# microsoft/Sora

Hardware: AMD Instinct MI355X
Metric: IQ Msamples/s through 802.11a 54 Mbps RX PHY (higher is better)
Workload: dtype int16 IQ / u8 path metrics

## Files before the change

### sora_amd/csrc/dev_vit16.h

```cpp
#pragma once
#include <hip/hip_runtime.h>
#include "kernels.h"
#include "dev_viterbi.h"

namespace sora {
namespace {

template <int WIN, int LOOK> struct Geom16 {
    static constexpr int kMaxWalk = (WIN + LOOK + 7) / 8 + 2;
    static constexpr int P = kMaxWalk;
    static constexpr int kPathBytes = 40;
};

template <int WIN, int LOOK> struct Lds16 {
    uint16_t ring[Geom16<WIN, LOOK>::P][4][64];
    union {
        uint32_t udump[4][64];
        uint16_t ops[4][24][2];
        uint16_t ops2[2][4][24][2];
    };
    uint8_t  path[8][Geom16<WIN, LOOK>::kPathBytes];
};

constexpr unsigned kW[4] = { 0u, 21u, 42u, 63u };

__device__ __forceinline__ unsigned v_of_lane(unsigned l)
{
    const unsigned b0 = l & 1u, b1 = (l >> 1) & 1u, b2 = (l >> 2) & 1u, b3 = (l >> 3) & 1u;
    const unsigned c3 = b2, c1 = b3, c0 = b0 ^ c3, c2 = b1 ^ c3;
    return c0 | (c1 << 1) | (c2 << 2) | (c3 << 3);
}
__device__ __forceinline__ unsigned lane_of_v(unsigned v)
{
    const unsigned c0 = v & 1u, c1 = (v >> 1) & 1u, c2 = (v >> 2) & 1u, c3 = (v >> 3) & 1u;
    return c0 ^ (c2 << 1) ^ (c1 << 3) ^ (c3 ? 7u : 0u);
}
__device__ __forceinline__ unsigned rev6u(unsigned x) { return __brev(x) >> 26; }

template <int CTRL> __device__ __forceinline__ unsigned dppx(unsigned v) { return (unsigned)__builtin_amdgcn_update_dpp(0, (int)v, CTRL, 0xF, 0xF, true); }

__device__ __forceinline__ unsigned partner(unsigned v, int ph)
{
    switch (ph) {
    case 0: return dppx<0x140>(v);
    case 1: return dppx<0x1B>(v);
    case 2: return dppx<0x141>(v);
    case 3: return dppx<0x4E>(v);
    case 4: return dppx<0x128>(v);
    default: return dppx<0xB1>(v);
    }
}

struct Vit16 {
    unsigned U[4];
    unsigned MX[24];
    unsigned MY[6];
    unsigned sadr[3][4];
};

template <int WHICH, int P>
__device__ __forceinline__ void acs16(Vit16& V, int t24, unsigned a, unsigned b, unsigned pos512[3])
{
    const int ph = t24 % 6, k = t24 % 8;
    const unsigned Kp = (WHICH == 0 ? 14u : 7u) * kFld + (kOne << k);
    unsigned bm;
    if (WHICH == 0)      bm = (a ^ V.MX[t24]) + (b ^ V.MY[ph]);
    else if (WHICH == 1) bm = a ^ V.MX[t24];
    else                 bm = b ^ V.MX[t24];
    const unsigned bo = Kp - bm;
    const int rx = ph == 0 ? 2 : ph == 1 ? 1 : 0;
    unsigned N[4];
#pragma unroll
    for (int i = 0; i < 4; i++) {
        const unsigned X = V.U[i], Y = partner(V.U[i ^ rx], ph);
        const bool wb = (kW[i] >> (5 - ph)) & 1u;
        N[i] = wb ? pk_min16(X + bo, Y + bm) : pk_min16(X + bm, Y + bo);
    }
#pragma unroll
    for (int i = 0; i < 4; i++) V.U[i] = N[i];
    if (k == 7) {
        const int jb = t24 / 8;
#pragma unroll
        for (int i = 0; i < 4; i++) {
            const unsigned w = bank_word(V.U[i]);
            const unsigned addr = V.sadr[jb][i] + pos512[jb];
            asm volatile("ds_write_b16 %0, %1" : : "v"(addr), "v"(w) : "memory");
            V.U[i] &= 0xFE00FE00u;
        }
    }
}

__device__ __forceinline__ unsigned row_min_u32(unsigned v)
{
    v = min(v, dppx<0xB1>(v)); v = min(v, dppx<0x4E>(v)); v = min(v, dppx<0x141>(v)); v = min(v, dppx<0x128>(v));
    return v;
}
__device__ __forceinline__ unsigned row_pkmin(unsigned v)
{
    v = pk_min16(v, dppx<0xB1>(v)); v = pk_min16(v, dppx<0x4E>(v)); v = pk_min16(v, dppx<0x141>(v)); v = pk_min16(v, dppx<0x128>(v));
    return v;
}
__device__ __forceinline__ unsigned wave_min_u32(unsigned v) { return (unsigned)__builtin_amdgcn_readfirstlane((int)dpp_min_u32_wave(v)); }
__device__ __forceinline__ unsigned wave_max_u32(unsigned v) { return ~wave_min_u32(~v); }

template <int CR, int WIN, int LOOK, int BITS>
struct Forward16 {
    static constexpr int P = Geom16<WIN, LOOK>::P, GB = Puncture<CR>::GB, GS = Puncture<CR>::GS, CW = Puncture<CR>::CW;
    static constexpr int NV = Puncture<CR>::NV;
    struct Chunk { uint32_t v[CW]; };
    struct Raw { SoftRaw r[NV]; };

    Vit16 V;
    unsigned row, half;
    uint32_t my_j;
    SoftCursor<BITS, CW> cur[NV];
    const uint8_t* soft;
    uint16_t* my_ops;
    const uint4* row_ops;
    uint32_t pos;
    unsigned pos512[3];
    uint32_t tr, nsteps;
    uint32_t next_thr;
    bool all_done;

    __device__ __forceinline__ void init(Lds16<WIN, LOOK>& S, const uint8_t* __restrict__ soft_, uint32_t my_soft_off, uint32_t my_first, uint32_t my_last, unsigned start,
                                         uint32_t nsteps_)
    {
        const unsigned lane = threadIdx.x & 63, l16 = lane & 15;
        row = lane >> 4; half = lane & 1u;
        const unsigned v0 = v_of_lane(l16);
        nsteps = nsteps_;
#pragma unroll
        for (int i = 0; i < 4; i++) V.U[i] = (v0 ^ kW[i]) == 0 ? 0u : start;
        const unsigned ring_base = (unsigned)(uintptr_t)&S.ring[0][0][0];
#pragma unroll
        for (int jb = 0; jb < 3; jb++)
#pragma unroll
            for (int i = 0; i < 4; i++) V.sadr[jb][i] = ring_base + ((row * 64u + rev6u(rol6(v0 ^ kW[i], jb == 0 ? 2 : jb == 1 ? 4 : 0))) << 1);
#pragma unroll
        for (int t = 0; t < 24; t++) {
            const int ph = t % 6, k = t % 8;
            const unsigned n = rol6(v0, ph + 1);
            const bool vb = (v0 >> (5 - ph)) & 1u;
            const unsigned ma = (__popc(n & 0155) & 1) ? 7u * kFld : 0u, mb = (__popc(n & 0117) & 1) ? 7u * kFld : 0u;
            const unsigned mx = Puncture<CR>::which_of(ph) == 2 ? mb : ma;
            V.MX[t] = vb ? ((mx ^ (7u * kFld)) | (kOne << k)) : mx;
            if (t < 6) V.MY[t] = vb ? (mb ^ (7u * kFld)) : mb;
        }
        tr = 0; pos = 0;
        my_j = l16 >> 1;
#pragma unroll
        for (int v = 0; v < NV; v++) cur[v].init(my_soft_off, my_first + my_j + 8u * v, my_last);
        soft = soft_;
        my_ops = &S.ops[row][my_j][half];
        row_ops = reinterpret_cast<const uint4*>(&S.ops[row][0][0]);
        set_row_pos();
    }
    __device__ __forceinline__ bool going() const { return tr < nsteps && !all_done; }

    __device__ __forceinline__ void normalize()
    {
        const unsigned m = row_pkmin(pk_min16(pk_min16(V.U[0], V.U[1]), pk_min16(V.U[2], V.U[3])));
#pragma unroll
        for (int i = 0; i < 4; i++) V.U[i] -= m;
    }
    static __device__ __forceinline__ uint32_t pos_of(uint32_t p, int jb) { const uint32_t q = p + (uint32_t)jb; return q >= (uint32_t)P ? q - (uint32_t)P : q; }
    __device__ __forceinline__ void set_row_pos()
    {
#pragma unroll
        for (int jb = 0; jb < 3; jb++) pos512[jb] = pos_of(pos, jb) * 512u;
    }
    __device__ __forceinline__ void end_row() { pos = pos_of(pos, 3); set_row_pos(); }
    __device__ __forceinline__ Raw fetch(uint32_t c) const
    {
        Raw R;
#pragma unroll
        for (int v = 0; v < NV; v++) R.r[v] = cur[v].fetch(soft, c);
        return R;
    }
    __device__ __forceinline__ void put(const Raw& R, uint16_t* mine) const
    {
#pragma unroll
        for (int v = 0; v < NV; v++) mine[16 * v] = (uint16_t)cur[v].field(R.r[v]);
    }
    static __device__ __forceinline__ Chunk get(const uint4* table)
    {
        Chunk K;
#pragma unroll
        for (int i = 0; i < (CW + 3) / 4; i++) {
            const uint4 x = table[i];
            K.v[4 * i] = x.x; K.v[4 * i + 1] = x.y;
            if (4 * i + 2 < CW) { K.v[4 * i + 2] = x.z; K.v[4 * i + 3] = x.w; }
        }
        return K;
    }
    __device__ __forceinline__ Chunk unpack(const Raw& R) const
    {
        put(R, my_ops);
        lds_fence();
        const Chunk K = get(row_ops);
        lds_fence();
        return K;
    }
    __device__ __forceinline__ void group(const Chunk& K, int h, int i0)
    {
        const int k0 = i0 / GS * GB, t24 = 12 * h + i0;
        acs16<0, P>(V, t24, K.v[k0], K.v[k0 + 1], pos512);
        if (CR != 0) acs16<1, P>(V, t24 + 1, K.v[k0 + 2], 0, pos512);
        if (CR == 2) acs16<2, P>(V, t24 + 2, 0, K.v[k0 + 3], pos512);
        if ((t24 + GS) % 8 == 0) normalize();
    }
    __device__ __forceinline__ void fast_chunk(const Chunk& K, int h)
    {
#pragma unroll
        for (int g = 0; g < 12 / GS; g++) group(K, h, g * GS);
        tr += 12;
    }
    template <typename CHECK> __device__ __forceinline__ void slow_chunk(const Chunk& K, int h, CHECK& check)
    {
#pragma unroll
        for (int g = 0; g < 12 / GS; g++) {
            if (going()) {
                group(K, h, g * GS);
                tr += GS;
                check(12 * h + g * GS + GS - 1);
            }
        }
    }
    template <typename CHECK> __device__ __forceinline__ void chunk(const Chunk& K, int h, CHECK& check)
    {
        if (tr + 12 <= nsteps && next_thr > tr + 12) fast_chunk(K, h); else slow_chunk(K, h, check);
    }
};

template <int WIN, int LOOK, bool LANE_OB = false>
__device__ __noinline__ void trace16(unsigned lds_off, unsigned U0, unsigned U1, unsigned U2, unsigned U3, uint32_t tr_, uint32_t ob_, uint32_t pj_, uint32_t k_,
                                     uint32_t my_cnt, uint8_t* my_out)
{
    using G = Geom16<WIN, LOOK>;
    constexpr int P = G::P;
    typedef __attribute__((address_space(3))) Lds16<WIN, LOOK> lds_t;
    lds_t& S = *(lds_t*)(uintptr_t)lds_off;
    auto uni = [](uint32_t v) { return (uint32_t)__builtin_amdgcn_readfirstlane((int)v); };
    const uint32_t tr = uni(tr_), ob = LANE_OB ? ob_ : uni(ob_), pj = uni(pj_), k = uni(k_);
    const unsigned lane = threadIdx.x & 63, row = lane >> 4, l16 = lane & 15, half = lane & 1u;
    const unsigned v0 = v_of_lane(l16);
    const unsigned U[4] = { U0, U1, U2, U3 };
    const uint32_t j = (tr - 1) >> 3, nn = tr - 8u * j, m_lo = ob >> 3;
#pragma unroll
    for (int i = 0; i < 4; i++) S.udump[i][lane] = U[i];
    lds_fence();
    unsigned key[2] = { 0xFFFFFFFFu, 0xFFFFFFFFu };
#pragma unroll
    for (int i = 0; i < 4; i++) {
        const unsigned st = rol6(v0 ^ kW[i], tr);
        unsigned lastA, lastB;
        if (k == 7) { const unsigned w = S.ring[pj][row][rev6u(st)]; lastA = (w >> 7) & 1u; lastB = (w >> 15) & 1u; }
        else { lastA = (U[i] >> k) & 1u; lastB = (U[i] >> (17 + k)) & 1u; }
        const unsigned mA = ((U[i] & 0xFFFFu) >> 9 << 1) | lastA, mB = (U[i] >> 25 << 1) | lastB;
        key[0] = min(key[0], (mA << 8) | (st << 2)); key[1] = min(key[1], (mB << 8) | (st << 2));
    }
    const unsigned kA = row_min_u32(key[0]), kB = row_min_u32(key[1]);
    const unsigned st = ((half ? kB : kA) >> 2) & 0x3Fu;
    const unsigned s0 = rol6(st, 6u - tr % 6u);
    const unsigned b4 = (s0 >> 4) & 1u, b5 = (s0 >> 5) & 1u;
    const unsigned ri = b4 | (b5 << 1);
    const unsigned sl = lane_of_v((s0 ^ (b4 ? 21u : 0u) ^ (b5 ? 42u : 0u)) & 15u);
    const unsigned Ust = S.udump[ri][row * 16u + sl];
    unsigned H;
    if (nn == 8) H = ((unsigned)S.ring[pj][row][rev6u(st)] >> (8u * half)) & 0xFFu;
    else H = ((Ust >> (17u * half)) & 0xFFu) & ((1u << nn) - 1u);
    unsigned q = rev6u(((st >> nn) | rev6u(H & 0x3Fu)) & 0x3Fu);
    __attribute__((address_space(3))) uint8_t* pth = S.path[row * 2u + half];
    pth[0] = (uint8_t)H;
    typedef __attribute__((address_space(3))) const uint16_t lds_u16;
    const unsigned rowbase = (unsigned)(uintptr_t)&S.ring[0][row][0], sh = 8u * half;
#pragma unroll
    for (int i = 1; i < G::kMaxWalk; i++) {
        const int d = (int)pj - i;
        const uint32_t p = (uint32_t)(d < 0 ? d + P : d);
        unsigned base = rowbase + p * 512u;
        asm volatile("" : "+v"(base));
        const unsigned raw = *(lds_u16*)(uintptr_t)(base + (q << 1));
        pth[i] = (uint8_t)(raw >> sh);
        q = __builtin_amdgcn_ubfe(raw, sh, 6u);
    }
    lds_fence();
    const uint32_t nbytes = my_cnt >> 3;
    for (uint32_t z = l16 >> 1; z < nbytes; z += 8) {
        const uint32_t m = m_lo + z, i1 = j - m;
        my_out[m] = (uint8_t)(((unsigned)pth[i1] >> 6) | (((unsigned)pth[i1 - 1] & 0x3Fu) << 2));
    }
    lds_fence();
}

}
}
```

### sora_amd/csrc/k_rx.hip

```cpp
#include <hip/hip_runtime.h>
#include <utility>
#include "kernels.h"
#include "dev_sym11a.h"
#include "dev_viterbi.h"
#include "dev_winplan.h"
#include "dev_vitwin.h"

namespace sora {

struct FrameLds {
    uint32_t eq[4][4][64];
    uint8_t  soft[4][4][288];
    uint8_t  demap[1024];
    int4     trk[4][4];
    int      nsym_of[4];
    short    st0[4][4];
};
template <bool SHARED>
__device__ __forceinline__ void frame_symbols(const RxArgs& A, uint32_t j, FrameLds& lds, bool valid = true)
{
    uint32_t (&s_eq)[4][4][64] = lds.eq; uint8_t (&s_soft)[4][4][288] = lds.soft; const uint8_t* s_demap = lds.demap;
    const int w = threadIdx.x >> 6, lane = threadIdx.x & 63, g = lane >> 4, e = lane & 15;
    const Tables& T = A.T;
    const uint32_t f = valid ? A.joblist[j] : 0u;
    FrameRow r = A.frames[f];
    if (!valid) { r.nsym = 0; r.nbpsc = 1; }
    if (lane == 0 && valid) A.jobs[j] = frame_vitjob(r);
    const FrameCtx* fx = A.fctx + f;
    const uint32_t* iq = A.iq + A.caps[r.capture].offset;
    const Fft64TwPk W = fft64_twiddles_pk(T, e);
    PkTw fq[4], ch[4];
#pragma unroll
    for (int m = 0; m < 4; m++) { fq[m] = pk_tw_mul(fx->freq[e + 16 * m]); ch[m] = pk_tw_mul(fx->chan[e + 16 * m]); }
    const int nb = __builtin_amdgcn_readfirstlane((int)r.nbpsc), ncbps = 48 * nb, nsym = __builtin_amdgcn_readfirstlane((int)r.nsym);
    uint32_t mp[4];
    const bool packs = deint_packs(nb, lane);
    deint_map_words(T, nb, lane, mp);
    uint8_t* dst = A.soft + (size_t)r.slot0 * kSoftBytesPerSlot;
    const int pk = lane & 3;
    const int pbin = pk == 0 ? 43 : pk == 1 ? 57 : pk == 2 ? 7 : 21, pc = pk == 0 ? -21 : pk == 1 ? -7 : pk == 2 ? 7 : 21;
    int cfo_comp = r.cfo_comp, sfo_comp = r.sfo_comp, cfo_tr = r.cfo_tracker, sfo_tr = r.sfo_tracker;
    unsigned symbol_count = 0;

    auto load_samples = [&](int s0, uint32_t raw[4]) {
        const uint32_t p0 = r.data_start + 80u * (uint32_t)(s0 + g) + 8u;
#pragma unroll
        for (int m = 0; m < 4; m++) raw[m] = (s0 + g <= nsym) ? iq[(size_t)(p0 + (uint32_t)(e + 16 * m)) * A.str] : 0u;
    };
    int nsym_loop = nsym, nsym_f = nsym;
    if (SHARED) {
        if (lane == 0) { lds.nsym_of[w] = nsym; lds.st0[w][0] = (short)cfo_comp; lds.st0[w][1] = (short)sfo_comp; lds.st0[w][2] = (short)cfo_tr; lds.st0[w][3] = (short)sfo_tr; }
        __syncthreads();
        nsym_loop = max(max(lds.nsym_of[0], lds.nsym_of[1]), max(lds.nsym_of[2], lds.nsym_of[3]));
        const int fr = (lane >> 2) & 3;
        nsym_f = lds.nsym_of[fr];
        cfo_comp = lds.st0[fr][0]; sfo_comp = lds.st0[fr][1]; cfo_tr = lds.st0[fr][2]; sfo_tr = lds.st0[fr][3];
    }
    uint32_t raw[4];
    load_samples(1, raw);
    for (int s0 = 1; s0 <= nsym_loop; s0 += 4) {
        const int sym = s0 + g;
        const bool active = sym <= nsym;
        const bool mine = s0 <= nsym;
        int4 rec = { 0, 0, 0, 0 };
        if (mine) {
            pcx x[4], Y[4];
#pragma unroll
            for (int m = 0; m < 4; m++) x[m] = sym_freq_comp(raw[m], fq[m]);
            if (s0 + 4 <= nsym) load_samples(s0 + 4, raw);
            fft64_core_pk(x, s_eq[w][g], e, W, wave_lds_sync);
#pragma unroll
            for (int q = 0; q < 4; q++) Y[q] = s_eq[w][g][__brev((unsigned)(e + 16 * q)) >> 26];
            wave_lds_sync();
#pragma unroll
            for (int q = 0; q < 4; q++) s_eq[w][g][e + 16 * q] = sym_equalise(Y[q], ch[q], e + 16 * q);
            wave_lds_sync();
        }
        if (SHARED) {
            __syncthreads();
            if (w == 0) {
                const int fr = (lane >> 2) & 3;
#pragma unroll
                for (int gg = 0; gg < 4; gg++) {
                    const cpx p = mul_q15(unpack(s_eq[fr][gg][pbin]), rot_coeff(T, w16(cfo_comp + pc * sfo_comp)));
                    const int th = pilot_angle(pk == 3 ? uatan2(T, -p.im, -p.re) : uatan2(T, p.im, p.re), (symbol_count + (unsigned)gg) % 127u);
                    int th1 = __builtin_amdgcn_update_dpp(0, th, 0x00, 0xF, 0xF, true), th2 = __builtin_amdgcn_update_dpp(0, th, 0x55, 0xF, 0xF, true);
                    int th3 = __builtin_amdgcn_update_dpp(0, th, 0xAA, 0xF, 0xF, true), th4 = __builtin_amdgcn_update_dpp(0, th, 0xFF, 0xF, 0xF, true);
                    asm volatile("" : "+v"(th1), "+v"(th2), "+v"(th3), "+v"(th4));
                    const int4 t = track_advance(th1, th2, th3, th4, s0 + gg <= nsym_f, cfo_comp, sfo_comp, cfo_tr, sfo_tr);
                    if (lane < 16 && pk == 0) lds.trk[fr][gg] = t;
                }
            }
            symbol_count = (symbol_count + 4u) % 127u;
            __syncthreads();
            rec = lds.trk[w][g];
        } else {
            int4 t[4];
#pragma unroll
            for (int gg = 0; gg < 4; gg++) {
                t[gg] = int4{ cfo_comp, sfo_comp, 0, 0 };
                if (s0 + gg <= nsym) {
                    const cpx p = mul_q15(unpack(s_eq[w][gg][pbin]), rot_coeff(T, w16(cfo_comp + pc * sfo_comp)));
                    const int th = pilot_angle(pk == 3 ? uatan2(T, -p.im, -p.re) : uatan2(T, p.im, p.re), symbol_count);
                    symbol_count++; if (symbol_count >= 127) symbol_count = 0;
                    t[gg] = track_advance(__builtin_amdgcn_readlane(th, 0), __builtin_amdgcn_readlane(th, 1), __builtin_amdgcn_readlane(th, 2), __builtin_amdgcn_readlane(th, 3),
                                          true, cfo_comp, sfo_comp, cfo_tr, sfo_tr);
                }
            }
            rec = t[0];
            if (g == 1) rec = t[1]; else if (g == 2) rec = t[2]; else if (g == 3) rec = t[3];
        }
        if (!mine) continue;
        if (active) {
            uint32_t v3[3];
#pragma unroll
            for (int m = 0; m < 3; m++) v3[m] = s_eq[w][g][carrier_bin48(e + 16 * m)];
            sym_back_demap(T, s_demap, v3, rec, nb, e, s_soft[w][g]);
        }
        wave_lds_sync();
        {
            const int nact = min(4, nsym - s0 + 1);
            const uint32_t sym_bytes = 3u * (uint32_t)ncbps / 8u;
            uint8_t* d = dst + (size_t)(s0 - 1) * sym_bytes;
            for (int gs = 0; gs < nact; gs++, d += sym_bytes)
                if (packs) soft3_store8(d, (uint32_t)lane, deint_gather24(s_soft[w][gs], mp));
        }
        wave_lds_sync();
    }
}
__global__ void __launch_bounds__(256) k_frame(RxArgs A)
{
    __shared__ FrameLds lds;
    reinterpret_cast<uint32_t*>(lds.demap)[threadIdx.x] = reinterpret_cast<const uint32_t*>(A.T.demap)[threadIdx.x];
    __syncthreads();
    if (!locate_job(blockIdx.x * 4, A.njobs).ok) return;
    const JobRef jr = locate_job(blockIdx.x * 4 + (threadIdx.x >> 6), A.njobs);
    frame_symbols<true>(A, jr.ok ? jr.list * A.nrows + jr.idx : 0u, lds, jr.ok);
}

typedef uint32_t u32x4_t __attribute__((ext_vector_type(4)));
__device__ __forceinline__ void store16_through(uint4* p, uint4 v)
{
    const u32x4_t x = { v.x, v.y, v.z, v.w };
    asm volatile("global_store_dwordx4 %0, %1, off sc1\n\ts_nop 1" : : "v"(p), "v"(x) : "memory");
}
__device__ __forceinline__ void store4_through(uint32_t* p, uint32_t v) { __hip_atomic_store(p, v, __ATOMIC_RELAXED, __HIP_MEMORY_SCOPE_AGENT); }

template <bool THROUGH>
__device__ __forceinline__ void sym_front_block(const RxArgs& A, uint32_t bid, uint32_t (*s_eq)[4][64])
{
    const int w = threadIdx.x >> 6, lane = threadIdx.x & 63, g = lane >> 4, e = lane & 15;
    const Tables& T = A.T;
    const WaveSlots S = wave_slots(A, bid);
    if (S.owned == 0) return;
    uint32_t own[kSlotIters];
#pragma unroll
    for (int it = 0; it < kSlotIters; it++) own[it] = S.owner(it, g);
    const Fft64TwPk W = fft64_twiddles_pk(T, e);
    uint32_t* sl = s_eq[w][g];
    uint4* eq4 = reinterpret_cast<uint4*>(A.eq);
    auto store = [&](uint32_t slot, const uint32_t o[4]) {
        if (THROUGH) store16_through(eq4 + ((size_t)slot * 16u + (uint32_t)e), uint4{ o[0], o[1], o[2], o[3] });
        else eq4[(size_t)slot * 16u + (uint32_t)e] = uint4{ o[0], o[1], o[2], o[3] };
        auto pilot = [&](uint32_t k, uint32_t v) { if (THROUGH) store4_through(A.pil + ((size_t)slot * 4u + k), v); else A.pil[(size_t)slot * 4u + k] = v; };
        if (e == 10) pilot(0u, o[3]);
        if (e == 14) pilot(1u, o[1]);
        if (e == 1)  pilot(2u, o[3]);
        if (e == 5)  pilot(3u, o[1]);
    };
    if (S.one_frame) {
        const FrameRow& r = A.frames[S.row0];
        const uint32_t* iq = A.iq + A.caps[r.capture].offset;
        const uint32_t ds = r.data_start, s0 = r.slot0, str = A.str;
        const FrameCtx* fx = A.fctx + S.row0;
        uint32_t raw[kSlotIters][4];
#pragma unroll
        for (int it = 0; it < kSlotIters; it++) {
            const uint32_t p0 = ds + 80u * (S.slot(it, g) - s0) + 8u;
#pragma unroll
            for (int m = 0; m < 4; m++) raw[it][m] = own[it] != kNoOwner ? iq[(size_t)(p0 + (uint32_t)(e + 16 * m)) * str] : 0u;
        }
        PkTw fq[4], ch[4];
#pragma unroll
        for (int m = 0; m < 4; m++) { fq[m] = pk_tw_mul(fx->freq[e + 16 * m]); ch[m] = pk_tw_mul(fx->chan[4 * e + m]); }
#pragma unroll
        for (int it = 0; it < kSlotIters; it++) {
            if (S.quad(it) == 0) continue;
            uint32_t o[4];
            sym_front_quad(raw[it], fq, ch, sl, e, W, o);
            if (own[it] != kNoOwner) store(S.slot(it, g), o);
        }
        return;
    }
#pragma unroll 1
    for (int it = 0; it < kSlotIters; it++) {
        if (S.quad(it) == 0) continue;
        const uint32_t ow = S.owner(it, g);
        const bool mine = ow != kNoOwner;
        const uint32_t slot = S.slot(it, g);
        uint32_t raw[4] = { 0u, 0u, 0u, 0u };
        PkTw fq[4], ch[4];
        const FrameCtx* fx = A.fctx + (mine ? ow : 0u);
        if (mine) {
            const FrameRow& r = A.frames[ow];
            const uint32_t* iq = A.iq + A.caps[r.capture].offset;
            const uint32_t p0 = r.data_start + 80u * (slot - r.slot0) + 8u;
#pragma unroll
            for (int m = 0; m < 4; m++) raw[m] = iq[(size_t)(p0 + (uint32_t)(e + 16 * m)) * A.str];
        }
#pragma unroll
        for (int m = 0; m < 4; m++) { fq[m] = pk_tw_mul(mine ? fx->freq[e + 16 * m] : 0u); ch[m] = pk_tw_mul(mine ? fx->chan[4 * e + m] : 0u); }
        uint32_t o[4];
        sym_front_quad(raw, fq, ch, sl, e, W, o);
        if (mine) store(slot, o);
    }
}

__global__ void __launch_bounds__(256) k_sym_front(RxArgs A)
{
    __shared__ uint32_t s_eq[4][4][64];
    sym_front_block<false>(A, blockIdx.x, s_eq);
}

__device__ __forceinline__ uint2 track_step(const TrkTables& s_t, uint32_t cur, int flip, int pc, int m3, int& cfo, int& sfo, int& ctr, int& str)
{
    constexpr float kInv28 = 0.0357142873108387f;
    const unsigned a = (unsigned)(cfo + pc * sfo) & 0xFFFFu;
    const int qi = trk_quarter_index(a);
    const int sraw = s_t.q[qi], craw = s_t.q[16384 - qi];
    const uint32_t ws = s_t.e2s[a >> 4], wc = s_t.e2c[a >> 4];
    const int ms = __builtin_amdgcn_sbfe((int)a, 15, 1), mc = __builtin_amdgcn_sbfe((int)(a ^ (a << 1)), 15, 1);
    const int sn = ((sraw ^ ms) - ms) + trk_sext2(ws, a), cs = ((craw ^ mc) - mc) + trk_sext2(wc, a);
    const int pr = (int)(short)cur, pi = (int)cur >> 16;
    const int re = __builtin_amdgcn_sbfe(pr * cs + pi * sn, 15, 16), im = __builtin_amdgcn_sbfe(pi * cs - pr * sn, 15, 16);
    const int x = (re ^ m3) - m3, y = (im ^ m3) - m3;
    const int sh = max(25 - __builtin_clz((unsigned)(max(x, -x) | max(y, -y)) | 1u), 0);
    int th = trk_uatan2_entry(s_t, y >> sh, x >> sh);
    th = __builtin_amdgcn_sbfe(th ^ flip, 0, 16);
    int th1, th2, th3, th4;
    asm volatile("s_nop 1\n\t"
                 "v_mov_b32_dpp %0, %4 quad_perm:[0,0,0,0] row_mask:0xf bank_mask:0xf bound_ctrl:1\n\t"
                 "v_mov_b32_dpp %1, %4 quad_perm:[1,1,1,1] row_mask:0xf bank_mask:0xf bound_ctrl:1\n\t"
                 "v_mov_b32_dpp %2, %4 quad_perm:[2,2,2,2] row_mask:0xf bank_mask:0xf bound_ctrl:1\n\t"
                 "v_mov_b32_dpp %3, %4 quad_perm:[3,3,3,3] row_mask:0xf bank_mask:0xf bound_ctrl:1"
                 : "=&v"(th1), "=&v"(th2), "=&v"(th3), "=&v"(th4) : "v"(th));
    const int sum = th1 + th2 + th3 + th4;
    const int avg = (sum + ((sum >> 31) & 3)) >> 2;
    const int del = ((int)((float)(th3 - th1) * kInv28) + (int)((float)(th4 - th2) * kInv28)) >> 1;
    const uint2 rec = uint2{ __builtin_amdgcn_perm((uint32_t)sfo, (uint32_t)cfo, 0x05040100u), __builtin_amdgcn_perm((uint32_t)del, (uint32_t)avg, 0x05040100u) };
    ctr += avg >> 2; str += del >> 2;
    cfo = (int)((unsigned)cfo + (unsigned)avg + (unsigned)ctr); sfo = __builtin_amdgcn_sbfe(sfo + del + str, 0, 16);
    return rec;
}

__device__ __forceinline__ void track_tables_to_lds(const uint32_t* __restrict__ trk, TrkTables& s_t, uint32_t* s_pol)
{
    if (threadIdx.x < 127) {
        unsigned b = 0;
#pragma unroll
        for (unsigned u = 0; u < 8; u++) b |= pilot_sgn((threadIdx.x + u) % 127u) << u;
        s_pol[threadIdx.x] = b;
    }
    const uint4* src = reinterpret_cast<const uint4*>(trk);
    uint4* dst = reinterpret_cast<uint4*>(&s_t);
    constexpr uint32_t kWords = sizeof(TrkTables) / 16, kBatch = 11;
    for (uint32_t i0 = threadIdx.x; i0 < kWords; i0 += 256u * kBatch) {
        uint4 v[kBatch];
#pragma unroll
        for (uint32_t b = 0; b < kBatch; b++) v[b] = src[min(i0 + 256u * b, kWords - 1u)];
#pragma unroll
        for (uint32_t b = 0; b < kBatch; b++) if (i0 + 256u * b < kWords) dst[i0 + 256u * b] = v[b];
    }
}

__global__ void __launch_bounds__(256) k_track_lds(RxArgs A)
{
    __shared__ TrkTables s_t;
    __shared__ uint32_t s_pol[128];
    track_tables_to_lds(A.T.trk, s_t, s_pol);
    __syncthreads();
    const int lane = threadIdx.x & 63, pk = lane & 3;
    const JobRef jr = locate_job(blockIdx.x * 64u + (threadIdx.x >> 2), A.njobs);
    const uint32_t j = jr.ok ? jr.list * A.nrows + jr.idx : 0u;
    const uint32_t f = jr.ok ? A.joblist[j] : 0u;
    const FrameRow r = A.frames[f];
    const int nsym = jr.ok ? (int)r.nsym : 0;
    if (jr.ok && pk == 0) A.jobs[j] = frame_vitjob(r);
    const int pc = pk == 0 ? -21 : pk == 1 ? -7 : pk == 2 ? 7 : 21;
    const int m3 = pk == 3 ? -1 : 0;
    int cfo = r.cfo_comp, sfo = r.sfo_comp, ctr = r.cfo_tracker, str = r.sfo_tracker;
    int nmax = nsym;
#pragma unroll
    for (int o = 32; o >= 4; o >>= 1) nmax = max(nmax, __shfl_xor(nmax, o));
    nmax = __builtin_amdgcn_readfirstlane(nmax);
    const uint32_t w0 = (jr.ok ? (r.slot0 + 1u) * 4u + (uint32_t)pk : (uint32_t)pk) * 4u;
    const uint32_t t0 = (jr.ok ? r.slot0 + 1u : A.total_slots + 1u) * 8u;
    const char* __restrict__ pil = reinterpret_cast<const char*>(A.pil);
    char* __restrict__ trk2 = reinterpret_cast<char*>(A.track);
    const unsigned last = (unsigned)max(nsym, 1) - 1u, nrec = (unsigned)nsym;
    constexpr int kAhead = 8;
    uint32_t q[kAhead];
#pragma unroll
    for (int i = 0; i < kAhead; i++) q[i] = *reinterpret_cast<const uint32_t*>(pil + (w0 + 16u * min((unsigned)i, last)));
    unsigned cnt = 0;
    for (int s0 = 1; s0 <= nmax; s0 += kAhead) {
        const unsigned pol = (unsigned)__builtin_amdgcn_readfirstlane((int)s_pol[cnt]);
        cnt = cnt + (unsigned)kAhead >= 127u ? cnt + (unsigned)kAhead - 127u : cnt + (unsigned)kAhead;
#pragma unroll
        for (int u = 0; u < kAhead; u++) {
            const int s = s0 + u;
            const uint32_t cur = q[u];
            q[u] = *reinterpret_cast<const uint32_t*>(pil + (w0 + 16u * min((unsigned)(s + kAhead - 1), last)));
            const int flip = (int)((pol << (15 - u)) & 0x8000u);
            *reinterpret_cast<uint2*>(trk2 + (t0 + 8u * min((unsigned)(s - 1), nrec))) = track_step(s_t, cur, flip, pc, m3, cfo, sfo, ctr, str);
        }
    }
}

__global__ void __launch_bounds__(256) k_sym_back(RxArgs A)
{
    __shared__ uint8_t s_soft[4][4][288];
    __shared__ uint8_t s_demap[1024];
    const int w = threadIdx.x >> 6, lane = threadIdx.x & 63, g = lane >> 4, e = lane & 15;
    const Tables& T = A.T;
    reinterpret_cast<uint32_t*>(s_demap)[threadIdx.x] = reinterpret_cast<const uint32_t*>(T.demap)[threadIdx.x];
    __syncthreads();
    const WaveSlots S = wave_slots(A, blockIdx.x);
    if (S.owned == 0) return;
    int bins[3];
#pragma unroll
    for (int m = 0; m < 3; m++) bins[m] = carrier_bin48(e + 16 * m);
    if (S.one_frame) {
        const FrameRow& r = A.frames[S.row0];
        const int nb = __builtin_amdgcn_readfirstlane((int)r.nbpsc), ncbps = 48 * nb;
        const uint32_t slot0 = (uint32_t)__builtin_amdgcn_readfirstlane((int)r.slot0), sym_bytes = 3u * (uint32_t)ncbps / 8u;
        uint8_t* stream = A.soft + (size_t)slot0 * kSoftBytesPerSlot;
        const bool packs = deint_packs(nb, lane);
        uint32_t mp[4];
        deint_map_words(T, nb, lane, mp);
        TrackRec tr[kSlotIters]; uint32_t v3[kSlotIters][3];
#pragma unroll
        for (int it = 0; it < kSlotIters; it++) {
            const uint32_t slot = S.slot(it, g);
            const bool mine = (S.quad(it) >> g) & 1u;
            tr[it] = mine ? A.track[slot] : TrackRec{ 0, 0, 0, 0 };
#pragma unroll
            for (int m = 0; m < 3; m++) v3[it][m] = mine ? A.eq[(size_t)slot * 64u + (uint32_t)bins[m]] : 0u;
        }
#pragma unroll
        for (int it = 0; it < kSlotIters; it++) {
            const unsigned quad = S.quad(it);
            if (quad == 0) continue;
            if ((quad >> g) & 1u) sym_back_demap(T, s_demap, v3[it], track_rec4(tr[it]), nb, e, s_soft[w][g]);
            wave_lds_sync();
#pragma unroll
            for (int gs = 0; gs < 4; gs++) {
                if (!((quad >> gs) & 1u) || !packs) continue;
                const uint32_t sg = S.slot(it, gs);
                soft3_store8(stream + (size_t)(sg - slot0 - 1u) * sym_bytes, (uint32_t)lane, deint_gather24(s_soft[w][gs], mp));
            }
            wave_lds_sync();
        }
// ... 598 lines not shown
```

Baseline: 52900.

## Pack Viterbi traceback bytes in registers and write decoded words directly

The traceback walk now keeps ring positions pre-scaled by 512 and wraps them with a subtract-and-select instead of multiply and compare. The decoded path bytes are packed into registers with byte-permute, and whole aligned windows are written straight to global memory as 32-bit words via alignbit, bypassing the per-byte LDS path buffer. Only partial windows still take the LDS fallback. Sample loading clamps the symbol index and replaces the stride multiply with a shift, which assumes the stride is 1 or 2 and the index fits in 32 bits.

```diff
diff --git a/sora_amd/csrc/dev_vit16.h b/sora_amd/csrc/dev_vit16.h
--- a/sora_amd/csrc/dev_vit16.h
+++ b/sora_amd/csrc/dev_vit16.h
@@ -19,7 +19,7 @@
         uint16_t ops[4][24][2];
         uint16_t ops2[2][4][24][2];
     };
-    uint8_t  path[8][Geom16<WIN, LOOK>::kPathBytes];
+    uint32_t path[8][Geom16<WIN, LOOK>::kPathBytes / 4];
 };
 
 constexpr unsigned kW[4] = { 0u, 21u, 42u, 63u };
@@ -164,13 +164,12 @@
 #pragma unroll
         for (int i = 0; i < 4; i++) V.U[i] -= m;
     }
-    static __device__ __forceinline__ uint32_t pos_of(uint32_t p, int jb) { const uint32_t q = p + (uint32_t)jb; return q >= (uint32_t)P ? q - (uint32_t)P : q; }
+    static __device__ __forceinline__ uint32_t pos_of(uint32_t p, int jb) { const uint32_t q = p + 512u * (uint32_t)jb; return min(q, q - 512u * (uint32_t)P); }
     __device__ __forceinline__ void set_row_pos()
     {
-#pragma unroll
-        for (int jb = 0; jb < 3; jb++) pos512[jb] = pos_of(pos, jb) * 512u;
-    }
-    __device__ __forceinline__ void end_row() { pos = pos_of(pos, 3); set_row_pos(); }
+        pos512[0] = pos; pos512[1] = pos_of(pos, 1); pos512[2] = pos_of(pos512[1], 1);
+    }
+    __device__ __forceinline__ void end_row() { pos = pos_of(pos512[2], 1); set_row_pos(); }
     __device__ __forceinline__ Raw fetch(uint32_t c) const
     {
         Raw R;
@@ -238,8 +237,12 @@
                                      uint32_t my_cnt, uint8_t* my_out)
 {
     using G = Geom16<WIN, LOOK>;
-    constexpr int P = G::P;
+    constexpr int P = G::P, K = G::kMaxWalk;
+    constexpr int NR = K - 1, NF = NR / 4, NW = K / 4 + 1;
+    static_assert(NR % 4 == 0 || NR % 4 == 2, "the walk's words are packed in pairs");
+    static_assert(NW * 4 <= G::kPathBytes && NW >= WIN / 32 + 1, "the stream's registers hold a window and fit Lds16::path");
     typedef __attribute__((address_space(3))) Lds16<WIN, LOOK> lds_t;
+    typedef __attribute__((address_space(3))) const uint16_t lds_u16;
     lds_t& S = *(lds_t*)(uintptr_t)lds_off;
     auto uni = [](uint32_t v) { return (uint32_t)__builtin_amdgcn_readfirstlane((int)v); };
     const uint32_t tr = uni(tr_), ob = LANE_OB ? ob_ : uni(ob_), pj = uni(pj_), k = uni(k_);
@@ -247,6 +250,8 @@
     const unsigned v0 = v_of_lane(l16);
     const unsigned U[4] = { U0, U1, U2, U3 };
     const uint32_t j = (tr - 1) >> 3, nn = tr - 8u * j, m_lo = ob >> 3;
+    const unsigned rowbase = (unsigned)(uintptr_t)&S.ring[0][row][0], sh = 8u * half;
+    auto ring_j = [&](unsigned idx) -> unsigned { return *(lds_u16*)(uintptr_t)(rowbase + pj + (idx << 1)); };
 #pragma unroll
     for (int i = 0; i < 4; i++) S.udump[i][lane] = U[i];
     lds_fence();
@@ -255,7 +260,7 @@
     for (int i = 0; i < 4; i++) {
         const unsigned st = rol6(v0 ^ kW[i], tr);
         unsigned lastA, lastB;
-        if (k == 7) { const unsigned w = S.ring[pj][row][rev6u(st)]; lastA = (w >> 7) & 1u; lastB = (w >> 15) & 1u; }
+        if (k == 7) { const unsigned w = ring_j(rev6u(st)); lastA = (w >> 7) & 1u; lastB = (w >> 15) & 1u; }
         else { lastA = (U[i] >> k) & 1u; lastB = (U[i] >> (17 + k)) & 1u; }
         const unsigned mA = ((U[i] & 0xFFFFu) >> 9 << 1) | lastA, mB = (U[i] >> 25 << 1) | lastB;
         key[0] = min(key[0], (mA << 8) | (st << 2)); key[1] = min(key[1], (mB << 8) | (st << 2));
@@ -268,31 +273,56 @@
     const unsigned sl = lane_of_v((s0 ^ (b4 ? 21u : 0u) ^ (b5 ? 42u : 0u)) & 15u);
     const unsigned Ust = S.udump[ri][row * 16u + sl];
     unsigned H;
-    if (nn == 8) H = ((unsigned)S.ring[pj][row][rev6u(st)] >> (8u * half)) & 0xFFu;
+    if (nn == 8) H = (ring_j(rev6u(st)) >> sh) & 0xFFu;
     else H = ((Ust >> (17u * half)) & 0xFFu) & ((1u << nn) - 1u);
     unsigned q = rev6u(((st >> nn) | rev6u(H & 0x3Fu)) & 0x3Fu);
-    __attribute__((address_space(3))) uint8_t* pth = S.path[row * 2u + half];
-    pth[0] = (uint8_t)H;
-    typedef __attribute__((address_space(3))) const uint16_t lds_u16;
-    const unsigned rowbase = (unsigned)(uintptr_t)&S.ring[0][row][0], sh = 8u * half;
-#pragma unroll
-    for (int i = 1; i < G::kMaxWalk; i++) {
-        const int d = (int)pj - i;
-        const uint32_t p = (uint32_t)(d < 0 ? d + P : d);
-        unsigned base = rowbase + p * 512u;
+    unsigned pr[NR / 2];
+    uint32_t p = pj;
+#pragma unroll
+    for (int i = 1; i < K; i++) {
+        uint32_t d;
+        p = __builtin_sub_overflow(p, 512u, &d) ? 512u * (uint32_t)(P - 1) : d;
+        unsigned base = rowbase + p;
         asm volatile("" : "+v"(base));
         const unsigned raw = *(lds_u16*)(uintptr_t)(base + (q << 1));
-        pth[i] = (uint8_t)(raw >> sh);
         q = __builtin_amdgcn_ubfe(raw, sh, 6u);
+        const int s = K - 1 - i;
+        if (s & 1) pr[s >> 1] = raw << 16; else pr[s >> 1] |= raw;
+    }
+    unsigned R[NW];
+    const unsigned sel = 0x06040200u + 0x01010101u * half;
+#pragma unroll
+    for (int w = 0; w < NF; w++) R[w] = __builtin_amdgcn_perm(pr[2 * w + 1], pr[2 * w], sel);
+    if (NR % 4 == 0) R[NF] = H;
+    else R[NF] = __builtin_amdgcn_perm(H, pr[2 * NF], 0x0C040200u + 0x00000101u * half);
+    const uint32_t sfirst = (uint32_t)(K - 1) - (j - m_lo);
+    bool fast = !LANE_OB;
+    if (!LANE_OB) {
+        const bool whole = my_cnt == (uint32_t)WIN && sfirst == 1u && (((uintptr_t)my_out + m_lo) & 3u) == 0;
+        fast = __ballot(!(whole || my_cnt == 0)) == 0;
+    }
+    if (fast) {
+        if (my_cnt != 0 && l16 < 2) {
+            uint32_t* o = reinterpret_cast<uint32_t*>(my_out + m_lo);
+#pragma unroll
+            for (int dw = 0; dw < WIN / 32; dw++) o[dw] = __builtin_amdgcn_alignbit(R[dw + 1], R[dw], 14);
+        }
+    } else {
+        __attribute__((address_space(3))) uint32_t* pw = S.path[row * 2u + half];
+        if (l16 < 2) {
+#pragma unroll
+            for (int w = 0; w < NW; w++) pw[w] = R[w];
+        }
+        lds_fence();
+        __attribute__((address_space(3))) const uint8_t* pth = (__attribute__((address_space(3))) const uint8_t*)pw;
+        const uint32_t nbytes = my_cnt >> 3;
+        for (uint32_t z = l16 >> 1; z < nbytes; z += 8) {
+            const uint32_t sb = sfirst + z;
+            my_out[m_lo + z] = (uint8_t)(((unsigned)pth[sb] >> 6) | (((unsigned)pth[sb + 1] & 0x3Fu) << 2));
+        }
     }
     lds_fence();
-    const uint32_t nbytes = my_cnt >> 3;
-    for (uint32_t z = l16 >> 1; z < nbytes; z += 8) {
-        const uint32_t m = m_lo + z, i1 = j - m;
-        my_out[m] = (uint8_t)(((unsigned)pth[i1] >> 6) | (((unsigned)pth[i1 - 1] & 0x3Fu) << 2));
-    }
-    lds_fence();
-}
-
-}
-}
+}
+
+}
+}
diff --git a/sora_amd/csrc/k_rx.hip b/sora_amd/csrc/k_rx.hip
--- a/sora_amd/csrc/k_rx.hip
+++ b/sora_amd/csrc/k_rx.hip
@@ -42,10 +42,11 @@
     int cfo_comp = r.cfo_comp, sfo_comp = r.sfo_comp, cfo_tr = r.cfo_tracker, sfo_tr = r.sfo_tracker;
     unsigned symbol_count = 0;
 
+    const uint32_t str_shift = A.str >> 1;
     auto load_samples = [&](int s0, uint32_t raw[4]) {
-        const uint32_t p0 = r.data_start + 80u * (uint32_t)(s0 + g) + 8u;
-#pragma unroll
-        for (int m = 0; m < 4; m++) raw[m] = (s0 + g <= nsym) ? iq[(size_t)(p0 + (uint32_t)(e + 16 * m)) * A.str] : 0u;
+        const uint32_t p0 = r.data_start + __umul24(80u, (uint32_t)min(s0 + g, nsym)) + 8u + (uint32_t)e;
+#pragma unroll
+        for (int m = 0; m < 4; m++) raw[m] = iq[(p0 + 16u * (uint32_t)m) << str_shift];
     };
     int nsym_loop = nsym, nsym_f = nsym;
     if (SHARED) {
@@ -56,8 +57,8 @@
         nsym_f = lds.nsym_of[fr];
         cfo_comp = lds.st0[fr][0]; sfo_comp = lds.st0[fr][1]; cfo_tr = lds.st0[fr][2]; sfo_tr = lds.st0[fr][3];
     }
-    uint32_t raw[4];
-    load_samples(1, raw);
+    uint32_t raw[4] = { 0u, 0u, 0u, 0u };
+    if (1 <= nsym) load_samples(1, raw);
     for (int s0 = 1; s0 <= nsym_loop; s0 += 4) {
         const int sym = s0 + g;
         const bool active = sym <= nsym;
```

Result: faster. 54080 (median of 6 runs) (+2.2%).
